# MMAThijssen/catfish

Hardware: AMD Instinct MI355X
Metric: signal samples/s classified (higher is better)
Workload: dtype f32

## Files before the change

### catfish_amd/csrc/catfish_hip.hip

```cpp
#include <hip/hip_runtime.h>
#include <stdint.h>
#include <string.h>
#include <stdio.h>
#include <vector>
#include <string>
#include <cmath>
#include <mutex>
#include <set>
#include <functional>

#include "../../include/catfish_hip.h"

typedef float f32x4 __attribute__((ext_vector_type(4)));
typedef float f32x2 __attribute__((ext_vector_type(2)));

#define CF_T 35
#define CF_H 64
#define CF_C 32
#define CF_TILE 16

#define MFMA16(a, b, c) __builtin_amdgcn_mfma_f32_16x16x4f32((a), (b), (c), 0, 0, 0)

#ifndef CF_ABLATE
#define CF_ABLATE 0
// ... 565 lines not shown
                cf_handoff_wait_agent(gflag - 1, lane, err);
            }
        }
        gru_tile<CIN, LAST, false, true>(lds, lane, dir, tile, X, Y, P, n_tiles, nullptr, nullptr, cf_dropout(), s_begin, s_end, ho, skip0);
        if (s_end < CF_T) {
            if (wave < nwaves - 1) cf_handoff_publish(flags + wave);
            else cf_handoff_publish_agent(gflag);
        }
    }
}

struct cf_fused_args {
    const float* w[3];
    const f32x4* x0;
    f32x4* y[2];
    float* p;
    unsigned* flags;
    int lds_floats;
    unsigned* err;
    int n_tiles;
    int groups;
    int n_layers;
    int cin0;
};

__device__ __forceinline__ bool cf_wait_flag(unsigned* flag) {
    for (int it = 0; it < 1000000; ++it) {
        if (__hip_atomic_load(flag, __ATOMIC_RELAXED, __HIP_MEMORY_SCOPE_AGENT) != 0u) return true;
        __builtin_amdgcn_s_sleep(16);
    }
    return false;
}

template <int CIN, bool LAST>
__device__ __forceinline__ void gru_fused_worker(float* lds, const cf_fused_args& a, int layer, int dir) {
    const f32x4* X = layer == 0 ? a.x0 : a.y[(layer - 1) & 1];
    f32x4* Y = a.y[layer & 1];
    gru_stage_weights<CIN>(lds, a.w[layer], dir);
    volatile int* slot = reinterpret_cast<volatile int*>(lds + a.lds_floats);
    unsigned* queue = a.flags + (size_t)a.n_layers * a.groups * 2 + layer * 2 + dir;
    const int lane = threadIdx.x & 63;
    const int wave = __builtin_amdgcn_readfirstlane(threadIdx.x >> 6);
    int group = 0;
    for (int iter = 0; iter <= a.groups && group < a.groups; ++iter) {
        if (threadIdx.x == 0) {
            const int g = (int)__hip_atomic_fetch_add(queue, 1u, __ATOMIC_RELAXED, __HIP_MEMORY_SCOPE_AGENT);
            if (layer > 0 && g < a.groups) {
                unsigned* f = a.flags + ((size_t)(layer - 1) * a.groups + g) * 2;
                if (!cf_wait_flag(f) || !cf_wait_flag(f + 1)) __hip_atomic_store(a.err, 1u, __ATOMIC_RELAXED, __HIP_MEMORY_SCOPE_SYSTEM);
                __builtin_amdgcn_fence(__ATOMIC_ACQUIRE, "agent");
                asm volatile("s_waitcnt vmcnt(0)" ::: "memory");
            }
            *slot = g;
        }
        __syncthreads();
        group = *slot;
        if (group < a.groups) {
            const int tile = group * 8 + wave;
            if (tile < a.n_tiles) gru_tile<CIN, LAST>(lds, lane, dir, tile, X, Y, a.p, a.n_tiles);
            asm volatile("s_waitcnt vmcnt(0)" ::: "memory");
            __syncthreads();
            if (!LAST && threadIdx.x == 0) {
                __builtin_amdgcn_fence(__ATOMIC_RELEASE, "agent");
                asm volatile("s_waitcnt vmcnt(0)" ::: "memory");
                __hip_atomic_store(a.flags + ((size_t)layer * a.groups + group) * 2 + dir, 1u, __ATOMIC_RELAXED,
                                   __HIP_MEMORY_SCOPE_AGENT);
            }
        }
    }
}

__global__ __launch_bounds__(512, 2) void gru_fused_kernel(cf_fused_args a) {
    extern __shared__ __attribute__((aligned(16))) float lds[];
    const int per_layer = gridDim.x / a.n_layers;
    const int layer = blockIdx.x / per_layer;
    const int dir = (blockIdx.x - layer * per_layer) & 1;
    const bool last = layer == a.n_layers - 1;
    if (layer == 0) {
        if (a.cin0 == 16) { if (last) gru_fused_worker<16, true>(lds, a, layer, dir); else gru_fused_worker<16, false>(lds, a, layer, dir); }
        else { if (last) gru_fused_worker<32, true>(lds, a, layer, dir); else gru_fused_worker<32, false>(lds, a, layer, dir); }
    } else {
        if (last) gru_fused_worker<128, true>(lds, a, layer, dir); else gru_fused_worker<128, false>(lds, a, layer, dir);
    }
}

#include "gru_coop.hpp"
#include "gru_train.hpp"
static_assert(gtb_pack_floats(32) == ((32 + CF_H) / 16 / 2) * 128 * 48 && gtb_pack_floats(128) == ((128 + CF_H) / 16 / 2) * 128 * 48,
              "gru_train_bwd_coop_kernel's PACK must equal gtb_pack_floats");
#include "gru_wgrad.hpp"
#include "res_train.hpp"
#include "train_step.hpp"

__global__ __launch_bounds__(256) void embed_kernel(const float* __restrict__ x_nat, f32x4* __restrict__ y_frag,
                                                    int64_t n_windows, int n_tiles) {
    const int64_t idx = (int64_t)blockIdx.x * 256 + threadIdx.x;
    if (idx >= (int64_t)n_tiles * CF_T * 64) return;
    const int lane = (int)(idx & 63);
    const int64_t tt = idx >> 6;
    const int t = (int)(tt % CF_T);
    const int64_t w = (tt / CF_T) * CF_TILE + (lane & 15);
    f32x4 v = {0.f, 0.f, 0.f, 0.f};
    if ((lane >> 4) == 0 && w < n_windows) v.x = x_nat[w * CF_T + t];
    y_frag[idx] = v;
}

#include "gru_bf16.hpp"
#include "gru_bf16_pipe.hpp"
#include "gru_bf16x3_pipe.hpp"

__global__ __launch_bounds__(256) void head_kernel(const float* __restrict__ P, const float* __restrict__ dense_bias, float* __restrict__ probs,
                                                   float* __restrict__ logits, int64_t n_windows, int n_tiles, int tile_shift, int raw) {
    const int64_t idx = (int64_t)blockIdx.x * 256 + threadIdx.x;
    if (idx >= n_windows * CF_T) return;
    const float bias = dense_bias[0];
// ... 225 lines not shown
        if (e_ != hipSuccess)                                                                      \
            return fail(CF_ERR_HIP, std::string(#expr) + ": " + hipGetErrorString(e_));           \
    } while (0)

enum { SLOT_RES_FIRST = 0, SLOT_RES, SLOT_GRU0, SLOT_GRU, SLOT_GRU_LAST, SLOT_HEAD, SLOT_POST, SLOT_NORM, SLOT_GRU_FUSED, SLOT_RES_STACK2 };
static const char* k_slot_names[CF_PROF_SLOTS] = {"res_block_first", "res_block",      "gru_layer_first", "gru_layer_mid",
                                                  "gru_layer_last",  "head",           "postprocess",     "normalize",       "gru_fused",
                                                  "res_stack2",      "unused",         "unused"};

struct cf_param_map;
static void pm_destroy(cf_param_map* pm);

struct cf_model {
    cf_hparams hp;
    int device = 0;
    int n_cu = 256;
    std::vector<float*> d_res;
    std::vector<float*> d_gru;
    std::vector<int> gru_cin;
    std::vector<char*> d_res_b;
    std::vector<char*> d_gru_b;
    int np = 0;
    float* d_dense_bias = nullptr;
    cf_param_map* pmap = nullptr;
    int64_t cap_windows = 0;
    int64_t cap_tiles = 0;
    struct Slot {
        float* d_a[2] = {nullptr, nullptr};
        float* d_y[2] = {nullptr, nullptr};
        float* d_p = nullptr;
        unsigned* d_flags = nullptr;
        float* d_hand = nullptr;
        unsigned* d_hand_flags = nullptr;
        hipStream_t stream = nullptr;
        hipEvent_t done = nullptr;
        int64_t last_windows = 0;
        bool last_res_fused = false;
    };
    std::vector<Slot> slots;
    cf_generic* gen = nullptr;
    int fuse = 0;
    float* d_xp = nullptr;
    int xp_tiles = 0;
    float* d_host_x = nullptr;
    float* d_host_p = nullptr;
    size_t host_stage_bytes = 0;
    unsigned* h_err = nullptr;
    unsigned* d_err = nullptr;
    hipEvent_t fork = nullptr;
    int64_t ws_bytes = 0;
    bool prof = false;
    int prof_every = 0;
    int64_t prof_calls = 0;
    struct Ev { hipEvent_t a, b; int slot; };
    std::vector<Ev> ev_pending;
    std::vector<hipEvent_t> ev_pool;
    double prof_ms[CF_PROF_SLOTS] = {0};
    int64_t prof_n[CF_PROF_SLOTS] = {0};
};

enum { CF_TERM_ZERO = 0, CF_TERM_RAW = 1, CF_TERM_KERN = 2, CF_TERM_BIAS = 3 };
enum { CF_K_ONE = 0, CF_K_GATE = 1, CF_K_CAND = 2 };
__host__ __device__ inline double cf_term_const(int c) { return c == CF_K_GATE ? CF_GATE_SCALE : (c == CF_K_CAND ? CF_CAND_SCALE : 1.0); }

__host__ __device__ inline double cf_bn_scale(float gamma, float var, float eps) {
#pragma clang fp contract(off)
// ... 210 lines not shown

static void pack_gru_dir(const cf_gru_dir& g, int cin, int cin_real, const float* dense_w ,
                         float* out) {
    cf_host_params P;
    P.t = {g.gates_kernel, g.gates_bias, g.candidate_kernel, g.candidate_bias, dense_w};
    HostSink e{P, out};
    pack_gru_dir(e, 0, gru_terms(0, CF_H), cin, cin_real, dense_w ? 4 : -1, 0);
}

static int upload(const std::vector<float>& host, float** dev) {
    HIP_TRY(hipMalloc((void**)dev, host.size() * sizeof(float)));
    HIP_TRY(hipMemcpy(*dev, host.data(), host.size() * sizeof(float), hipMemcpyHostToDevice));
    return CF_OK;
}

static bool gen_wanted(const cf_hparams* hp);
static int gen_build(cf_model* m, const cf_weights* w);
static void gen_destroy(cf_generic* g);
static hipError_t cf_optin_all();

extern "C" void cf_model_destroy(cf_model* m) {
    if (!m) return;
    (void)hipSetDevice(m->device);
    for (float* p : m->d_res) if (p) (void)hipFree(p);
    for (float* p : m->d_gru) if (p) (void)hipFree(p);
    for (char* p : m->d_gru_b) if (p) (void)hipFree(p);
    for (char* p : m->d_res_b) if (p) (void)hipFree(p);
    for (auto& sl : m->slots) {
        for (int i = 0; i < 2; ++i) { if (sl.d_a[i]) (void)hipFree(sl.d_a[i]); if (sl.d_y[i]) (void)hipFree(sl.d_y[i]); }
        if (sl.d_p) (void)hipFree(sl.d_p);
        if (sl.d_flags) (void)hipFree(sl.d_flags);
        if (sl.d_hand) (void)hipFree(sl.d_hand);
        if (sl.d_hand_flags) (void)hipFree(sl.d_hand_flags);
        if (sl.stream) (void)hipStreamDestroy(sl.stream);
        if (sl.done) (void)hipEventDestroy(sl.done);
    }
    gen_destroy(m->gen);
    pm_destroy(m->pmap);
    if (m->d_dense_bias) (void)hipFree(m->d_dense_bias);
    if (m->d_xp) (void)hipFree(m->d_xp);
    if (m->d_host_x) (void)hipFree(m->d_host_x);
    if (m->h_err) (void)hipHostFree(m->h_err);
    if (m->fork) (void)hipEventDestroy(m->fork);
    for (auto& e : m->ev_pending) { (void)hipEventDestroy(e.a); (void)hipEventDestroy(e.b); }
    for (auto& e : m->ev_pool) (void)hipEventDestroy(e);
    delete m;
}

extern "C" int cf_model_create(const cf_weights* w, const cf_hparams* hp, int device, cf_model** out) {
    if (!w || !hp || !out) return fail(CF_ERR_INVALID, "cf_model_create: null argument");
    *out = nullptr;
    if (hp->window != CF_T) return fail(CF_ERR_INVALID, "window must be 35 (rnn_class.py:27)");
    if (hp->n_layers < 1 || hp->n_layers_res < 0) return fail(CF_ERR_INVALID, "n_layers must be >= 1 and n_layers_res >= 0");
    const bool generic = gen_wanted(hp);
    if (!generic && hp->n_layers_res == 0 && hp->precision != CF_PREC_FP32)
        return fail(CF_ERR_INVALID, "the plain RNN type (n_layers_res = 0) is only built for CF_PREC_FP32");
    if ((hp->n_layers_res > 0 && !w->conv) || !w->gru || !w->dense_kernel || !w->dense_bias)
        return fail(CF_ERR_INVALID, "cf_weights has null members");
    int n_dev = 0;
    HIP_TRY(hipGetDeviceCount(&n_dev));
    if (device < 0 || device >= n_dev) return fail(CF_ERR_INVALID, "device index out of range");
    HIP_TRY(hipSetDevice(device));

    if (hp->precision < CF_PREC_FP32 || hp->precision > CF_PREC_BF16)
        return fail(CF_ERR_INVALID, "precision must be CF_PREC_FP32, CF_PREC_BF16X3 or CF_PREC_BF16");
    cf_model* m = new cf_model();
// ... 40 lines not shown
        if (w->gru[2 * l].cin != cin_real || w->gru[2 * l + 1].cin != cin_real) { rc = fail(CF_ERR_INVALID, "GRU layer input width mismatch"); break; }
        const bool last = l == hp->n_layers - 1;
        std::vector<float> blob((size_t)2 * gru_pack_floats(cin));
        HostSink e{P, blob.data()};
        for (int d = 0; d < 2; ++d)
            pack_gru_dir(e, (size_t)d * gru_pack_floats(cin), gru_terms(cf_tid_gru(hp->n_layers_res, l, d, 0), CF_H), cin, cin_real,
                         last ? cf_tid_dense(hp->n_layers_res, hp->n_layers, 0) : -1, d * CF_H);
        float* dptr = nullptr;
        rc = upload(blob, &dptr);
        m->d_gru.push_back(dptr);
        m->gru_cin.push_back(cin);
        if (rc == CF_OK && m->np > 0) {
            const size_t bytes = (size_t)gb_pack_bytes(cin, m->np);
            std::vector<char> bblob(2 * bytes, 0);
            for (int d = 0; d < 2; ++d)
                pack_gru_dir_bf16(w->gru[2 * l + d], cin, m->np, last ? w->dense_kernel + d * CF_H : nullptr, bblob.data() + d * bytes);
            char* bptr = nullptr;
            hipError_t e = hipMalloc((void**)&bptr, bblob.size());
            if (e == hipSuccess) e = hipMemcpy(bptr, bblob.data(), bblob.size(), hipMemcpyHostToDevice);
            if (e != hipSuccess) rc = fail(CF_ERR_HIP, std::string("bf16 weight upload: ") + hipGetErrorString(e));
            m->d_gru_b.push_back(bptr);
        }
    }
    if (rc == CF_OK) {
        int64_t cap = hp->max_windows_per_pass > 0 ? hp->max_windows_per_pass : 32768;
        cap = (cap + 2 * CF_TILE - 1) / (2 * CF_TILE) * (2 * CF_TILE);
        m->cap_windows = cap;
        m->cap_tiles = cap / CF_TILE;
        const size_t a_bytes = (size_t)m->cap_tiles * CF_T * 2 * 64 * sizeof(f32x4);
        const size_t y_bytes = (size_t)m->cap_tiles * CF_T * 8 * 64 * sizeof(f32x4);
        const cf_knobs knobs = cf_read_knobs();
        const size_t p_bytes = cf_dense_partial_floats(m->cap_tiles, m->n_cu) * sizeof(float);
        const size_t hand_bytes = cf_hand_bytes(m->n_cu);
        hipError_t e = hipSuccess;
        int n_slots = hp->n_streams > 0 ? hp->n_streams : 1;
        if (n_slots > 8) n_slots = 8;
        m->slots.resize(n_slots);
        for (auto& sl : m->slots) {
            for (int i = 0; i < 2 && e == hipSuccess; ++i) e = hipMalloc((void**)&sl.d_a[i], a_bytes);
            for (int i = 0; i < 2 && e == hipSuccess; ++i) e = hipMalloc((void**)&sl.d_y[i], y_bytes);
            if (e == hipSuccess) e = hipMalloc((void**)&sl.d_p, p_bytes);
            if (e == hipSuccess) e = hipMalloc((void**)&sl.d_flags, (size_t)3 * ((m->cap_tiles + 7) / 8) * 2 * sizeof(unsigned) + 64);
            if (e == hipSuccess && m->np == 0) e = hipMalloc((void**)&sl.d_hand, hand_bytes);
            if (e == hipSuccess && m->np == 0) e = hipMalloc((void**)&sl.d_hand_flags, cf_hand_flag_bytes(m->n_cu));
            if (e == hipSuccess && m->np == 0) e = hipMemset(sl.d_hand_flags, 0, cf_hand_flag_bytes(m->n_cu));
            if (e == hipSuccess && n_slots > 1) e = hipStreamCreateWithFlags(&sl.stream, hipStreamNonBlocking);
            if (e == hipSuccess && n_slots > 1) e = hipEventCreateWithFlags(&sl.done, hipEventDisableTiming);
        }
        if (e == hipSuccess && n_slots > 1) e = hipEventCreateWithFlags(&m->fork, hipEventDisableTiming);
        if (e == hipSuccess && n_slots == 1 && m->np == 0) {
            const int xpt = cf_hoist_limit(m->n_cu, m->cap_tiles, knobs);
            e = hipMalloc((void**)&m->d_xp, cf_xp_floats(xpt) * sizeof(float));
            if (e == hipSuccess) m->xp_tiles = xpt;
        }
        if (e == hipSuccess) e = hipHostMalloc((void**)&m->h_err, sizeof(unsigned), hipHostMallocMapped);
        if (e == hipSuccess) { *m->h_err = 0u; e = hipHostGetDevicePointer((void**)&m->d_err, m->h_err, 0); }
        m->fuse = cf_fuse_mode(m->np == 0 && hp->n_layers <= 3, hp->fuse_layers, knobs);
        if (e != hipSuccess) rc = fail(CF_ERR_NOMEM, std::string("workspace allocation: ") + hipGetErrorString(e));
        m->ws_bytes = (int64_t)n_slots * (int64_t)(2 * a_bytes + 2 * y_bytes + p_bytes + (m->np == 0 ? hand_bytes : 0));
    }
    if (rc == CF_OK) {
        hipError_t e = cf_optin_all();
        if (e != hipSuccess) rc = fail(CF_ERR_HIP, std::string("hipFuncSetAttribute(max dynamic LDS): ") + hipGetErrorString(e));
    }
    if (rc != CF_OK) { std::string keep = g_err; cf_model_destroy(m); g_err = keep; return rc; }
    *out = m;
    return CF_OK;
}

static int prof_begin(cf_model* m, int slot, hipStream_t s, size_t* idx) {
    if (!m->prof) return CF_OK;
    cf_model::Ev ev;
    ev.slot = slot;
    for (hipEvent_t* p : {&ev.a, &ev.b}) {
        if (!m->ev_pool.empty()) { *p = m->ev_pool.back(); m->ev_pool.pop_back(); }
        else HIP_TRY(hipEventCreate(p));
    }
    HIP_TRY(hipEventRecord(ev.a, s));
    m->ev_pending.push_back(ev);
    *idx = m->ev_pending.size() - 1;
    return CF_OK;
}
static int prof_end(cf_model* m, hipStream_t s, size_t idx) {
    if (!m->prof) return CF_OK;
    HIP_TRY(hipEventRecord(m->ev_pending[idx].b, s));
    return CF_OK;
}

template <int... Vs, class F>
static int cf_with(int v, F&& f) {
    int rc = CF_OK;
    const bool hit = ((v == Vs && ((rc = f(std::integral_constant<int, Vs>{})), true)) || ...);
    return hit ? rc : fail(CF_ERR_INVALID, "no kernel is built for template argument " + std::to_string(v));
}

struct cf_optin {
    hipError_t e = hipSuccess;
    void operator()(const void* f, int bytes) { if (e == hipSuccess) e = hipFuncSetAttribute(f, hipFuncAttributeMaxDynamicSharedMemorySize, bytes); }
};

template <int CIN> constexpr int k_gru_pack_bytes = gru_pack_floats(CIN) * 4;
template <int CIN> constexpr int k_gru_x_bytes = gru_x_floats(CIN) * 4;
static void optin_gru_layer(cf_optin& o) {
    for (int cin : {16, 32, 128})
        for (int last : {0, 1})
            cf_with<16, 32, 128>(cin, [&](auto C) { return cf_with<0, 1>(last, [&](auto L) {
                constexpr int CIN = decltype(C)::value;
                constexpr bool LAST = decltype(L)::value != 0;
                o((const void*)gru_layer_kernel<CIN, LAST>, cf_gru_layer_lds(k_gru_pack_bytes<CIN>));
                o((const void*)gru_layer_coop_kernel<CIN, LAST>, cf_gru_coop_lds(k_gru_pack_bytes<CIN>));
                return CF_OK;
            }); });
    o((const void*)gru_fused_kernel, cf_fused_lds(k_gru_pack_bytes<128>));
    o((const void*)gru_xproj_lds_kernel<32>, k_gru_x_bytes<32>);
    o((const void*)gru_xproj_lds_kernel<128>, k_gru_x_bytes<128>);
}

template <int CIN>
static void launch_xproj(cf_model* m, const cf_xproj_launch& xp, const float* wpack, const float* X, int n_tiles, hipStream_t s) {
    if (xp.lds_kernel)
        hipLaunchKernelGGL((gru_xproj_lds_kernel<CIN>), dim3(xp.grid_x, 2), dim3(256), xp.lds_bytes, s, wpack,
                           reinterpret_cast<const f32x4*>(X), reinterpret_cast<f32x4*>(m->d_xp), n_tiles, xp.chunks);
    else
        hipLaunchKernelGGL((gru_xproj_kernel<CIN>), dim3(xp.grid_x, 2), dim3(256), 0, s, wpack,
                           reinterpret_cast<const f32x4*>(X), reinterpret_cast<f32x4*>(m->d_xp), n_tiles, xp.chunks);
}

static int launch_gru(cf_model* m, const cf_knobs& k, int cin, bool last, const float* wpack, const float* X, float* Y, float* P, int n_tiles,
                      hipStream_t s, int slot, cf_gru_plan* ran = nullptr,
                      float* hand = nullptr,
                      unsigned* hand_flags = nullptr) {
    return cf_with<16, 32, 128>(cin, [&](auto C) { return cf_with<0, 1>(last, [&](auto L) {
        constexpr int CIN = decltype(C)::value;
        constexpr bool LAST = decltype(L)::value != 0;
        const cf_gru_plan p = cf_gru_plan_for(n_tiles, m->n_cu, CIN, k_gru_pack_bytes<CIN>, k_gru_x_bytes<CIN>, m->xp_tiles, hand && hand_flags, k);
        if (ran) *ran = p;
        size_t pi = 0;
        int rc = prof_begin(m, slot, s, &pi);
        if (rc != CF_OK) return rc;
        if (p.coop) {
            if (p.hoist) launch_xproj<CIN>(m, p.xproj, wpack, X, n_tiles, s);
            hipLaunchKernelGGL((gru_layer_coop_kernel<CIN, LAST>), dim3(p.gx, 2), dim3(p.waves * 64), p.lds_bytes, s, wpack,
                               reinterpret_cast<const f32x4*>(X), reinterpret_cast<f32x4*>(Y), P, n_tiles,
                               p.hoist ? reinterpret_cast<const f32x4*>(m->d_xp) : nullptr);
        } else {
            hipLaunchKernelGGL((gru_layer_kernel<CIN, LAST>), dim3(p.gx, 2), dim3(p.waves * 64), p.lds_bytes, s, wpack,
// ... 106 lines not shown
            if ((rc = prof_begin(m, b == 0 ? SLOT_RES_FIRST : SLOT_RES, s, &pi)) != CF_OK) return rc;
            bf16x8* dst = reinterpret_cast<bf16x8*>(sl.d_a[b & 1]);
            if (b == 0)
                hipLaunchKernelGGL((res_block_bf16_kernel<true, NP>), dim3(p.grid), dim3(256), p.lds_first, s, m->d_res_b[0], x, (const bf16x8*)nullptr,
                                   dst, n_windows, n_tiles32);
            else
                hipLaunchKernelGGL((res_block_bf16_kernel<false, NP>), dim3(p.grid), dim3(256), p.lds_other, s, m->d_res_b[b], (const float*)nullptr,
                                   reinterpret_cast<const bf16x8*>(sl.d_a[(b - 1) & 1]), dst, n_windows, n_tiles32);
            HIP_TRY(hipGetLastError());
            if ((rc = prof_end(m, s, pi)) != CF_OK) return rc;
        }
        return CF_OK;
    });
}

static int run_pass(cf_model* m, cf_model::Slot& sl, const float* x, int64_t n_windows, float* probs, float* logits, hipStream_t s) {
    const int n_tiles = (int)((n_windows + CF_TILE - 1) / CF_TILE);
    const int n_tiles32 = (int)((n_windows + 2 * CF_TILE - 1) / (2 * CF_TILE));
    const cf_knobs k = cf_read_knobs();
    int rc;
    size_t pi = 0;
    if ((rc = m->np > 0 ? run_res_bf16(m, sl, k, x, n_windows, n_tiles32, s) : run_res_fp32(m, sl, k, x, n_windows, n_tiles, s)) != CF_OK) return rc;
    if (m->hp.n_layers_res == 0) {
        if ((rc = prof_begin(m, SLOT_RES_FIRST, s, &pi)) != CF_OK) return rc;
        const int64_t n_el = (int64_t)n_tiles * CF_T * 64;
        hipLaunchKernelGGL(embed_kernel, dim3((unsigned)((n_el + 255) / 256)), dim3(256), 0, s, x,
                           reinterpret_cast<f32x4*>(sl.d_a[0]), n_windows, n_tiles);
        HIP_TRY(hipGetLastError());
        if ((rc = prof_end(m, s, pi)) != CF_OK) return rc;
    }
    const float* cur = m->hp.n_layers_res == 0 ? sl.d_a[0] : sl.d_a[(m->hp.n_layers_res - 1) & 1];
    cf_gru_plan last_gru = {};
    const int cin0 = m->hp.n_layers_res == 0 ? 16 : CF_C;
    if (cf_fuse_now(m->fuse, n_tiles, m->n_cu)) {
        cf_fused_args a;
        a.lds_floats = m->hp.n_layers > 1 ? gru_pack_floats(128) : gru_pack_floats(cin0);
        const cf_fused_plan p = cf_fused_plan_for(n_tiles, m->n_cu, m->hp.n_layers, a.lds_floats * 4);
        for (int l = 0; l < 3; ++l) a.w[l] = l < m->hp.n_layers ? m->d_gru[l] : nullptr;
        a.x0 = reinterpret_cast<const f32x4*>(cur);
        a.y[0] = reinterpret_cast<f32x4*>(sl.d_y[0]);
        a.y[1] = reinterpret_cast<f32x4*>(sl.d_y[1]);
        a.p = sl.d_p;
        a.flags = sl.d_flags;
        a.err = m->d_err;
        a.n_tiles = n_tiles;
        a.groups = p.groups;
        a.n_layers = m->hp.n_layers;
        a.cin0 = cin0;
        HIP_TRY(hipMemsetAsync(sl.d_flags, 0, ((size_t)a.n_layers * a.groups * 2 + (size_t)a.n_layers * 2) * sizeof(unsigned), s));
        if ((rc = prof_begin(m, SLOT_GRU_FUSED, s, &pi)) != CF_OK) return rc;
        hipLaunchKernelGGL(gru_fused_kernel, dim3((unsigned)p.grid), dim3(p.threads), p.lds_bytes, s, a);
        HIP_TRY(hipGetLastError());
        if ((rc = prof_end(m, s, pi)) != CF_OK) return rc;
    } else {
        for (int l = 0; l < m->hp.n_layers; ++l) {
            const bool last = l == m->hp.n_layers - 1;
            const int slot = last ? SLOT_GRU_LAST : (l == 0 ? SLOT_GRU0 : SLOT_GRU);
            float* y = sl.d_y[l & 1];
            rc = m->np > 0 ? launch_gru_bf16(m, k, m->gru_cin[l], last, m->d_gru_b[l], cur, y, sl.d_p, n_tiles32, s, slot)
                           : launch_gru(m, k, m->gru_cin[l], last, m->d_gru[l], cur, y, sl.d_p, n_tiles, s, slot, &last_gru, sl.d_hand, sl.d_hand_flags);
            if (rc != CF_OK) return rc;
            cur = y;
        }
    }
    if ((rc = prof_begin(m, SLOT_HEAD, s, &pi)) != CF_OK) return rc;
    const int64_t total = n_windows * CF_T;
    hipLaunchKernelGGL(head_kernel, dim3((unsigned)((total + 255) / 256)), dim3(256), 0, s, sl.d_p, m->d_dense_bias, probs, logits, n_windows,
                       m->np > 0 ? n_tiles32 : n_tiles, m->np > 0 ? 5 : 4, last_gru.raw_partials);
    HIP_TRY(hipGetLastError());
    if ((rc = prof_end(m, s, pi)) != CF_OK) return rc;
    sl.last_windows = n_windows;
    return CF_OK;
}

static const char* k_fused_timeout_msg = "a fused biGRU launch timed out waiting for a producer workgroup; its results are invalid "
                                         "(create the model with fuse_layers = -1)";

extern "C" int cf_check_error(cf_model* m) {
    if (!m) return fail(CF_ERR_INVALID, "cf_check_error: null model");
    if (m->h_err && *m->h_err) return fail(CF_ERR_HIP, k_fused_timeout_msg);
    return CF_OK;
}

extern "C" int cf_clear_error(cf_model* m) {
    if (!m) return fail(CF_ERR_INVALID, "cf_clear_error: null model");
    if (m->h_err) *m->h_err = 0u;
    HIP_TRY(hipSetDevice(m->device));
    HIP_TRY(hipDeviceSynchronize());
    for (auto& sl : m->slots)
        if (sl.d_hand_flags) HIP_TRY(hipMemset(sl.d_hand_flags, 0, cf_hand_flag_bytes(m->n_cu)));
    return CF_OK;
}

extern "C" int cf_launch_regimes(const cf_model* m, int64_t out[4]) {
    if (!m || !out) return fail(CF_ERR_INVALID, "cf_launch_regimes: null argument");
    out[0] = m->n_cu;
    if (m->gen) { out[1] = out[2] = out[3] = 0; return CF_OK; }
    out[1] = (int64_t)m->xp_tiles * CF_TILE;
    out[2] = m->np == 0 ? (int64_t)cf_coop_max_tiles(m->n_cu) * CF_TILE : 0;
    out[3] = m->fuse == 1 ? 1 : (m->fuse == 2 ? cf_fuse_auto_min_windows(m->n_cu) : 0);
    return CF_OK;
}

extern "C" int cf_infer_logits(cf_model* m, const float* x, int64_t n_windows, float* probs, float* logits, void* stream) {
    if (!m) return fail(CF_ERR_INVALID, "cf_infer: null model");
    if (n_windows < 0) return fail(CF_ERR_INVALID, "cf_infer: negative n_windows");
    if (n_windows == 0) return CF_OK;
    if (!x || (!probs && !logits)) return fail(CF_ERR_INVALID, "cf_infer: null buffer");
    if (m->h_err && *m->h_err) return fail(CF_ERR_HIP, k_fused_timeout_msg);
    HIP_TRY(hipSetDevice(m->device));
    hipStream_t s = reinterpret_cast<hipStream_t>(stream);
    m->prof = m->prof_every > 0 && (m->prof_calls++ % m->prof_every) == 0;
    if (m->gen) {
        for (int64_t off = 0; off < n_windows; off += m->cap_windows) {
            const int64_t n = std::min(m->cap_windows, n_windows - off);
            const int rc = gen_run_pass(m, x + off * CF_T, n, probs ? probs + off * CF_T : nullptr, logits ? logits + off * CF_T : nullptr, s);
            if (rc != CF_OK) return rc;
        }
        return CF_OK;
    }
    const int n_slots = (int)m->slots.size();
    int64_t chunk = m->cap_windows;
    if (n_slots > 1) {
// ... 827 lines not shown
```

### catfish_amd/csrc/gru_balance.hpp

```cpp
#pragma once

#if defined(__HIPCC__) || defined(__CUDACC__)
#define CF_BAL_HD __host__ __device__
#else
#define CF_BAL_HD
#endif

struct cf_gru_share {
    int head_tile, head_end;
    int whole_first, whole_count;
    int tail_tile, tail_begin;
    int interior;
    int steps;
};

CF_BAL_HD inline cf_gru_share cf_gru_balanced_share(int tiles, int nwaves, int wave, int T) {
    const int total = tiles * T;
    const int a = (int)((long long)wave * total / nwaves), b = (int)((long long)(wave + 1) * total / nwaves);
    cf_gru_share s;
    s.steps = b - a;
    s.tail_tile = a / T;
    s.tail_begin = a % T == 0 ? T : a % T;
    s.head_tile = b / T;
    s.head_end = b % T;
// ... 52 lines not shown
    int worst = 0;
    long long rem = 0;
    for (int b = 0; b < gx; ++b) {
        int big = 0;
        for (int w = 0; w < nwaves; ++w) {
            rem += r;
            if (rem >= W) { rem -= W; ++big; }
        }
        const int v = per_simd * q + (big < per_simd ? big : per_simd);
        if (v > worst) worst = v;
    }
    return worst * wg_per_cu;
}

struct cf_gru_choice {
    int balance;
    int gx;
    int load;
};
CF_BAL_HD inline cf_gru_choice cf_gru_choose(int n_tiles, int gx, int gx_one, int nwaves, int wg_per_cu, int T, int forced) {
    const bool two = gx_one > 0 && gx > gx_one;
    const int load_rr = cf_gru_grid_load(n_tiles, gx, nwaves, wg_per_cu, T, 0);
    const int load_bal = cf_gru_grid_load(n_tiles, gx, nwaves, wg_per_cu, T, 1);
    const int load_one = two ? cf_gru_grid_load(n_tiles, gx_one, nwaves, 1, T, 1) : -1;
    const int load_grid = cf_gru_gridwide_load(n_tiles, gx, nwaves, wg_per_cu, T);
    const int load_grid_one = two ? cf_gru_gridwide_load(n_tiles, gx_one, nwaves, 1, T) : -1;
    cf_gru_choice c = {0, gx, load_rr};
    if (forced < 0 ? (load_bal >= 0 && load_bal < c.load) : (forced >= 1 && load_bal >= 0)) { c.balance = 1; c.load = load_bal; }
    if (forced < 0 ? (load_one >= 0 && load_one < c.load) : (forced >= 2 && load_one >= 0)) { c.balance = 1; c.gx = gx_one; c.load = load_one; }
    if (forced < 0 ? (load_grid >= 0 && load_grid < c.load) : (forced == 3 && load_grid >= 0)) { c.balance = 2; c.gx = gx; c.load = load_grid; }
    if (forced < 0 ? (load_grid_one >= 0 && load_grid_one < c.load) : (forced == 3 && load_grid_one >= 0)) { c.balance = 2; c.gx = gx_one; c.load = load_grid_one; }
    return c;
}
```

### catfish_amd/csrc/tuned_launch.hpp

```cpp
#pragma once

#include <algorithm>
#include <climits>
#include <cstddef>
#include <cstdint>

#ifndef CF_T
#define CF_T 35
#define CF_TILE 16
#endif
#define CF_GRU_MAX_WAVES 8
#define CF_COOP_XCH_FLOATS (2 * 4 * 64 * 4 + 4 * 64)
#define CF_COOP_BWD_XCH_FLOATS (3 * 4 * 64 * 4)
#include "gru_balance.hpp"

constexpr int CF_LDS_LIMIT = 160 * 1024;
enum { CF_GRU_SCHED_MASK = 3, CF_GRU_RUN_ZERO_PRODUCTS = 4 };

constexpr int CF_KNOB_UNSET = INT_MIN;
struct cf_knobs {
    int coop = CF_KNOB_UNSET, waves = CF_KNOB_UNSET, gru_balance = CF_KNOB_UNSET, gru_gx = CF_KNOB_UNSET, gru_zero_products = CF_KNOB_UNSET;
    int xproj_lds = CF_KNOB_UNSET, xproj_chunks = CF_KNOB_UNSET, hoist_tiles = CF_KNOB_UNSET, fuse = CF_KNOB_UNSET;
    int bf16_waves = CF_KNOB_UNSET, bf16_wgs = CF_KNOB_UNSET, bf16_pipe = CF_KNOB_UNSET;
    int res_fuse = CF_KNOB_UNSET, res_tpw = CF_KNOB_UNSET, res_chunks = CF_KNOB_UNSET, dx_chunks = CF_KNOB_UNSET;
// ... 91 lines not shown
    int lds_bytes;
    int raw_partials;
};
inline cf_gru_plan cf_gru_plan_for(int n_tiles, int n_cu, int cin, int pack_bytes, int x_bytes, int hoist_tiles, bool has_hand, const cf_knobs& k) {
    cf_gru_plan p = {};
    p.load = -1;
    if (cf_use_coop(n_tiles, n_cu, k)) {
        p.coop = p.raw_partials = 1;
        p.waves = 4;
        p.gx = cf_coop_gx(n_tiles, n_cu);
        p.hoist = cin >= 32 && n_tiles <= hoist_tiles;
        if (p.hoist) p.xproj = cf_xproj_launch_for(n_tiles, n_cu, cin, x_bytes, k);
        p.lds_bytes = cf_gru_coop_lds(pack_bytes);
        return p;
    }
    const int gx_env = cf_forced_gx(n_cu, k);
    p.waves = gx_env > 0 ? 8 : k.waves > 0 ? std::min(k.waves, 8) : (k.ablate_four_waves ? 4 : cf_pick_waves(2 * n_tiles, n_cu));
    const int groups = cf_ceil_div(n_tiles, p.waves);
    p.per_dir = cf_half_cus(n_cu);
    if (pack_bytes <= CF_LDS_LIMIT / 2) p.per_dir *= 2;
    p.gx = std::min(groups, p.per_dir);
    if (gx_env > 0) p.gx = std::min(gx_env, groups);
    p.balance = CF_GRU_RUN_ZERO_PRODUCTS;
    if (has_hand) {
        p.wg_per_cu = std::max(1, cf_ceil_div(2 * p.gx, n_cu));
        p.gx_one = gx_env > 0 ? 0 : cf_half_cus(n_cu);
        const cf_gru_choice c = cf_gru_choose(n_tiles, p.gx, p.gx_one, p.waves, p.wg_per_cu, CF_T, cf_knob_or(k.gru_balance, -1));
        p.balance = c.balance | (cf_knob_or(k.gru_zero_products, 0) != 0 ? CF_GRU_RUN_ZERO_PRODUCTS : 0);
        p.gx = c.gx;
        p.load = c.load;
    }
    p.lds_bytes = cf_gru_layer_lds(pack_bytes);
    return p;
}

struct cf_gru_bf16_plan {
    int pipe;
    int waves, gx, lds_bytes;
};
inline cf_gru_bf16_plan cf_gru_bf16_plan_for(int n_tiles32, int n_cu, int np, int pack_bytes, const cf_knobs& k) {
    cf_gru_bf16_plan p;
    p.pipe = cf_knob_or(k.bf16_pipe, 1) != 0;
    p.lds_bytes = pack_bytes;
    p.waves = k.bf16_waves > 0 ? std::min(k.bf16_waves, 8) : cf_pick_waves(2 * n_tiles32, n_cu);
    int per_dir = cf_half_cus(n_cu);
    if (np == 2 && p.pipe) {
        p.waves = std::min(p.waves, 4);
    } else if (pack_bytes <= CF_LDS_LIMIT / 2) {
        per_dir *= 2;
    }
    if (k.bf16_wgs > 0) per_dir = k.bf16_wgs;
    p.gx = std::min(cf_ceil_div(n_tiles32, p.waves), per_dir);
    return p;
}

constexpr int CF_XS_BYTES = CF_TILE * CF_T * 4;
struct cf_res_plan {
    int split;
    int chunks, waves, grid;
    int lds_first, lds_other;
    int fused;
    int stack_chunks, stack_waves, stack_grid, stack_lds;
};
constexpr int cf_res_stack2_lds(int pack_first_bytes, int pack_other_bytes, int waves) { return pack_first_bytes + pack_other_bytes + waves * CF_XS_BYTES; }
inline cf_res_plan cf_res_plan_for(int n_tiles, int n_cu, int n_blocks, int pack_first_bytes, int pack_other_bytes, const cf_knobs& k) {
    cf_res_plan p = {};
// ... 88 lines not shown
```

Before: 348.4 million.

## Add chained multi-layer GRU kernel with per-producer epoch flags and fused head

Adds a single persistent kernel that runs all GRU layers and both directions at once. Each workgroup handles a fixed balanced share and waits only on the specific producer workgroups of the layer below, using epoch-tagged done flags, instead of a layer-wide barrier or separate launches. The last layer also computes the sigmoid head inline once both directions for a tile have arrived, which removes the separate head kernel launch. It is enabled automatically for fp32 models with up to three layers when the gridwide balanced plan applies. The cost is extra sync workspace and spin-waits, and it depends on every layer's workgroups being co-resident on the device.

```diff
diff --git a/catfish_amd/csrc/catfish_hip.hip b/catfish_amd/csrc/catfish_hip.hip
--- a/catfish_amd/csrc/catfish_hip.hip
+++ b/catfish_amd/csrc/catfish_hip.hip
@@ -621,6 +621,14 @@
     return false;
 }
 
+__device__ __forceinline__ bool cf_wait_flag_is(unsigned* flag, unsigned value) {
+    for (int it = 0; it < 1000000; ++it) {
+        if (__hip_atomic_load(flag, __ATOMIC_RELAXED, __HIP_MEMORY_SCOPE_AGENT) == value) return true;
+        __builtin_amdgcn_s_sleep(16);
+    }
+    return false;
+}
+
 template <int CIN, bool LAST>
 __device__ __forceinline__ void gru_fused_worker(float* lds, const cf_fused_args& a, int layer, int dir) {
     const f32x4* X = layer == 0 ? a.x0 : a.y[(layer - 1) & 1];
@@ -670,6 +678,134 @@
         else { if (last) gru_fused_worker<32, true>(lds, a, layer, dir); else gru_fused_worker<32, false>(lds, a, layer, dir); }
     } else {
         if (last) gru_fused_worker<128, true>(lds, a, layer, dir); else gru_fused_worker<128, false>(lds, a, layer, dir);
+    }
+}
+
+struct cf_chain_args {
+    const float* w[3];
+    const f32x4* x0;
+    f32x4* y[2];
+    float* p;
+    f32x4* hand;
+    unsigned* gflags;
+    unsigned* done;
+    unsigned* arrive;
+    unsigned* epoch;
+    const float* dense_bias;
+    float* probs;
+    unsigned* err;
+    long long n_windows;
+    int n_tiles, gx, n_layers, cin0;
+    int skip0;
+    int ablate;
+};
+
+template <int CIN, bool LAST>
+__device__ __forceinline__ void gru_chain_worker(float* lds, const cf_chain_args& a, int layer, int dir, int b) {
+    const f32x4* X = layer == 0 ? a.x0 : a.y[(layer - 1) & 1];
+    f32x4* Y = a.y[layer & 1];
+    gru_stage_weights<CIN>(lds, a.w[layer], dir);
+    unsigned* flags = reinterpret_cast<unsigned*>(lds + gru_pack_floats(CIN));
+    if (threadIdx.x <= CF_GRU_MAX_WAVES) flags[threadIdx.x] = 0u;
+    auto set_now = [&]() { return __hip_atomic_load(a.epoch, __ATOMIC_RELAXED, __HIP_MEMORY_SCOPE_AGENT) + 1u; };
+    const int lane = threadIdx.x & 63;
+    const int wave = __builtin_amdgcn_readfirstlane(threadIdx.x >> 6);
+    const int nwaves = blockDim.x >> 6;
+    if (layer > 0 && threadIdx.x == 0 && !(a.ablate & 4)) {
+        const cf_gru_wg_range r = cf_gru_chain_producers(a.n_tiles, a.gx, nwaves, CF_T, b, 0, 0);
+        unsigned* below = a.done + (size_t)(layer - 1) * 2 * a.gx;
+        const unsigned want = set_now();
+        bool ok = true;
+        for (int i = 0; i < r.count; ++i) {
+            const int pb = (r.first + i) % a.gx;
+            ok = cf_wait_flag_is(below + pb, want) && ok;
+            ok = cf_wait_flag_is(below + a.gx + pb, want) && ok;
+        }
+        if (!ok) __hip_atomic_store(a.err, 1u, __ATOMIC_RELAXED, __HIP_MEMORY_SCOPE_SYSTEM);
+        __builtin_amdgcn_fence(__ATOMIC_ACQUIRE, "agent");
+        asm volatile("s_waitcnt vmcnt(0)" ::: "memory");
+    }
+    __syncthreads();
+    const cf_gru_share sh = cf_gru_balanced_share(a.n_tiles, a.gx * nwaves, b * nwaves + wave, CF_T);
+    const int has_head = sh.head_end > 0;
+    const int n_pieces = has_head + sh.whole_count + (sh.tail_begin < CF_T);
+    const size_t row = (size_t)(layer * 2 + dir) * a.gx + b;
+    f32x4* slots = a.hand + row * CF_GRU_MAX_WAVES * 4 * 64;
+    unsigned* gflag = a.gflags + row;
+    const float bias = LAST ? a.dense_bias[0] : 0.f;
+    for (int i = 0; i < n_pieces; ++i) {
+        int tile, s_begin = 0, s_end = CF_T;
+        f32x4* ho = nullptr;
+        if (i < has_head) {
+            tile = sh.head_tile; s_end = sh.head_end; ho = slots + wave * 4 * 64;
+        } else if (i < has_head + sh.whole_count) {
+            tile = sh.whole_first + (i - has_head);
+        } else {
+            tile = sh.tail_tile; s_begin = sh.tail_begin;
+            if (wave > 0) {
+                ho = slots + (wave - 1) * 4 * 64;
+                cf_handoff_wait(flags + (wave - 1), lane, a.err);
+            } else {
+                ho = slots - (CF_GRU_MAX_WAVES - (nwaves - 1)) * 4 * 64;
+                cf_handoff_wait_agent(gflag - 1, lane, a.err);
+            }
+        }
+        gru_tile<CIN, LAST, false, true>(lds, lane, dir, tile, X, Y, a.p, a.n_tiles, nullptr, nullptr, cf_dropout(), s_begin, s_end, ho,
+                                         a.skip0 != 0);
+        if (s_end < CF_T) {
+            if (wave < nwaves - 1) cf_handoff_publish(flags + wave);
+            else cf_handoff_publish_agent(gflag);
+        } else if (LAST && a.probs) {
+            asm volatile("s_waitcnt vmcnt(0)" ::: "memory");
+            __builtin_amdgcn_fence(__ATOMIC_RELEASE, "agent");
+            asm volatile("s_waitcnt vmcnt(0)" ::: "memory");
+            unsigned before = 0u;
+            if (lane == 0) before = __hip_atomic_fetch_add(a.arrive + tile, 1u, __ATOMIC_RELAXED, __HIP_MEMORY_SCOPE_AGENT);
+            if (__builtin_amdgcn_readfirstlane(before) & 1u) {
+                __builtin_amdgcn_fence(__ATOMIC_ACQUIRE, "agent");
+                asm volatile("s_waitcnt vmcnt(0)" ::: "memory");
+                const float* pf = a.p + (int64_t)tile * CF_T * 16;
+                const float* pb = a.p + ((int64_t)a.n_tiles + tile) * CF_T * 16;
+                for (int j = lane; j < CF_TILE * CF_T; j += 64) {
+                    const int wl = j / CF_T, t = j - wl * CF_T;
+                    if ((int64_t)tile * CF_TILE + wl < a.n_windows) {
+                        const float z = pf[t * 16 + wl] + pb[t * 16 + wl] + bias;
+                        a.probs[(int64_t)tile * CF_TILE * CF_T + j] = 1.0f / (1.0f + expf(-z));
+                    }
+                }
+            }
+        }
+    }
+    if (!LAST && !(a.ablate & 2)) {
+        asm volatile("s_waitcnt vmcnt(0)" ::: "memory");
+        __builtin_amdgcn_fence(__ATOMIC_RELEASE, "agent");
+        asm volatile("s_waitcnt vmcnt(0)" ::: "memory");
+    }
+    if (lane == 0) {
+        const unsigned through = __hip_atomic_fetch_add(flags + CF_GRU_MAX_WAVES, 1u, __ATOMIC_ACQ_REL, __HIP_MEMORY_SCOPE_WORKGROUP);
+        if (through == (unsigned)nwaves - 1u) {
+            const unsigned set = set_now();
+            if constexpr (!LAST) __hip_atomic_store(a.done + row, set, __ATOMIC_RELAXED, __HIP_MEMORY_SCOPE_AGENT);
+            const unsigned out = __hip_atomic_fetch_add(a.epoch + 1, 1u, __ATOMIC_RELAXED, __HIP_MEMORY_SCOPE_AGENT);
+            if (out == gridDim.x - 1u) {
+                __hip_atomic_store(a.epoch + 1, 0u, __ATOMIC_RELAXED, __HIP_MEMORY_SCOPE_AGENT);
+                __hip_atomic_store(a.epoch, set, __ATOMIC_RELAXED, __HIP_MEMORY_SCOPE_AGENT);
+            }
+        }
+    }
+}
+
+__global__ __launch_bounds__(512, 2) void gru_chain_kernel(cf_chain_args a) {
+    extern __shared__ __attribute__((aligned(16))) float lds[];
+    const int layer = blockIdx.x / (2 * a.gx);
+    const int rest = blockIdx.x - layer * 2 * a.gx;
+    const int dir = rest / a.gx, b = rest - dir * a.gx;
+    const bool last = layer == a.n_layers - 1;
+    if (layer == 0) {
+        if (a.cin0 == 16) { if (last) gru_chain_worker<16, true>(lds, a, layer, dir, b); else gru_chain_worker<16, false>(lds, a, layer, dir, b); }
+        else { if (last) gru_chain_worker<32, true>(lds, a, layer, dir, b); else gru_chain_worker<32, false>(lds, a, layer, dir, b); }
+    } else {
+        if (last) gru_chain_worker<128, true>(lds, a, layer, dir, b); else gru_chain_worker<128, false>(lds, a, layer, dir, b);
     }
 }
 
@@ -961,6 +1097,8 @@
         unsigned* d_flags = nullptr;
         float* d_hand = nullptr;
         unsigned* d_hand_flags = nullptr;
+        float* d_chain_hand = nullptr;
+        unsigned* d_chain_sync = nullptr;
         hipStream_t stream = nullptr;
         hipEvent_t done = nullptr;
         int64_t last_windows = 0;
@@ -1237,6 +1375,8 @@
         if (sl.d_flags) (void)hipFree(sl.d_flags);
         if (sl.d_hand) (void)hipFree(sl.d_hand);
         if (sl.d_hand_flags) (void)hipFree(sl.d_hand_flags);
+        if (sl.d_chain_hand) (void)hipFree(sl.d_chain_hand);
+        if (sl.d_chain_sync) (void)hipFree(sl.d_chain_sync);
         if (sl.stream) (void)hipStreamDestroy(sl.stream);
         if (sl.done) (void)hipEventDestroy(sl.done);
     }
@@ -1343,6 +1483,7 @@
         const cf_knobs knobs = cf_read_knobs();
         const size_t p_bytes = cf_dense_partial_floats(m->cap_tiles, m->n_cu) * sizeof(float);
         const size_t hand_bytes = cf_hand_bytes(m->n_cu);
+        const bool chain_ws = m->np == 0 && hp->n_layers <= 3;
         hipError_t e = hipSuccess;
         int n_slots = hp->n_streams > 0 ? hp->n_streams : 1;
         if (n_slots > 8) n_slots = 8;
@@ -1355,6 +1496,9 @@
             if (e == hipSuccess && m->np == 0) e = hipMalloc((void**)&sl.d_hand, hand_bytes);
             if (e == hipSuccess && m->np == 0) e = hipMalloc((void**)&sl.d_hand_flags, cf_hand_flag_bytes(m->n_cu));
             if (e == hipSuccess && m->np == 0) e = hipMemset(sl.d_hand_flags, 0, cf_hand_flag_bytes(m->n_cu));
+            if (e == hipSuccess && chain_ws) e = hipMalloc((void**)&sl.d_chain_hand, cf_chain_hand_bytes(m->n_cu));
+            if (e == hipSuccess && chain_ws) e = hipMalloc((void**)&sl.d_chain_sync, cf_chain_sync_bytes(m->n_cu, m->cap_tiles));
+            if (e == hipSuccess && chain_ws) e = hipMemset(sl.d_chain_sync, 0, cf_chain_sync_bytes(m->n_cu, m->cap_tiles));
             if (e == hipSuccess && n_slots > 1) e = hipStreamCreateWithFlags(&sl.stream, hipStreamNonBlocking);
             if (e == hipSuccess && n_slots > 1) e = hipEventCreateWithFlags(&sl.done, hipEventDisableTiming);
         }
@@ -1368,7 +1512,8 @@
         if (e == hipSuccess) { *m->h_err = 0u; e = hipHostGetDevicePointer((void**)&m->d_err, m->h_err, 0); }
         m->fuse = cf_fuse_mode(m->np == 0 && hp->n_layers <= 3, hp->fuse_layers, knobs);
         if (e != hipSuccess) rc = fail(CF_ERR_NOMEM, std::string("workspace allocation: ") + hipGetErrorString(e));
-        m->ws_bytes = (int64_t)n_slots * (int64_t)(2 * a_bytes + 2 * y_bytes + p_bytes + (m->np == 0 ? hand_bytes : 0));
+        m->ws_bytes = (int64_t)n_slots * (int64_t)(2 * a_bytes + 2 * y_bytes + p_bytes + (m->np == 0 ? hand_bytes : 0) +
+                                                 (chain_ws ? cf_chain_hand_bytes(m->n_cu) : 0));
     }
     if (rc == CF_OK) {
         hipError_t e = cf_optin_all();
@@ -1423,6 +1568,7 @@
                 return CF_OK;
             }); });
     o((const void*)gru_fused_kernel, cf_fused_lds(k_gru_pack_bytes<128>));
+    o((const void*)gru_chain_kernel, cf_chain_lds(k_gru_pack_bytes<128>));
     o((const void*)gru_xproj_lds_kernel<32>, k_gru_x_bytes<32>);
     o((const void*)gru_xproj_lds_kernel<128>, k_gru_x_bytes<128>);
 }
@@ -1595,7 +1741,45 @@
     const float* cur = m->hp.n_layers_res == 0 ? sl.d_a[0] : sl.d_a[(m->hp.n_layers_res - 1) & 1];
     cf_gru_plan last_gru = {};
     const int cin0 = m->hp.n_layers_res == 0 ? 16 : CF_C;
-    if (cf_fuse_now(m->fuse, n_tiles, m->n_cu)) {
+    const char* chain_env = cf_knob("CATFISH_CHAIN");
+    const bool fuse_now = cf_fuse_now(m->fuse, n_tiles, m->n_cu);
+    const cf_chain_plan ch = cf_chain_plan_for(n_tiles, m->n_cu, m->hp.n_layers, cin0, cin0 == 16 ? k_gru_pack_bytes<16> : k_gru_pack_bytes<32>,
+                                               k_gru_pack_bytes<128>, cin0 == 16 ? k_gru_x_bytes<16> : k_gru_x_bytes<32>, k_gru_x_bytes<128>,
+                                               m->xp_tiles, m->np == 0 && sl.d_chain_hand && sl.d_chain_sync, logits != nullptr, m->prof,
+                                               chain_env ? atoi(chain_env) : CF_KNOB_UNSET, CF_CHAIN_AUTO && !fuse_now, k);
+    if (ch.on) {
+        cf_chain_args a;
+        for (int l = 0; l < 3; ++l) a.w[l] = l < m->hp.n_layers ? m->d_gru[l] : nullptr;
+        a.x0 = reinterpret_cast<const f32x4*>(cur);
+        a.y[0] = reinterpret_cast<f32x4*>(sl.d_y[0]);
+        a.y[1] = reinterpret_cast<f32x4*>(sl.d_y[1]);
+        a.p = sl.d_p;
+        a.hand = reinterpret_cast<f32x4*>(sl.d_chain_hand);
+        a.epoch = sl.d_chain_sync;
+        a.gflags = sl.d_chain_sync + 4;
+        a.done = a.gflags + cf_chain_max_rows(m->n_cu);
+        a.arrive = a.done + cf_chain_max_rows(m->n_cu);
+        a.dense_bias = m->d_dense_bias;
+        a.probs = probs;
+        a.err = m->d_err;
+        a.n_windows = n_windows;
+        a.n_tiles = n_tiles;
+        a.gx = ch.gx;
+        a.n_layers = m->hp.n_layers;
+        a.cin0 = cin0;
+        a.skip0 = ch.skip0;
+        const char* abl_env = cf_knob("CATFISH_CHAIN_ABLATE");
+        a.ablate = abl_env ? atoi(abl_env) : 0;
+        if (a.ablate & 1) a.probs = nullptr;
+        hipLaunchKernelGGL(gru_chain_kernel, dim3((unsigned)ch.grid), dim3(ch.threads), ch.lds_bytes, s, a);
+        HIP_TRY(hipGetLastError());
+        sl.last_windows = n_windows;
+        if (!(a.ablate & 1)) return CF_OK;
+        hipLaunchKernelGGL(head_kernel, dim3((unsigned)((n_windows * CF_T + 255) / 256)), dim3(256), 0, s, sl.d_p, m->d_dense_bias, probs, logits, n_windows,
+                           n_tiles, 4, 0);
+        return CF_OK;
+    }
+    if (fuse_now) {
         cf_fused_args a;
         a.lds_floats = m->hp.n_layers > 1 ? gru_pack_floats(128) : gru_pack_floats(cin0);
         const cf_fused_plan p = cf_fused_plan_for(n_tiles, m->n_cu, m->hp.n_layers, a.lds_floats * 4);
@@ -1652,6 +1836,8 @@
     HIP_TRY(hipDeviceSynchronize());
     for (auto& sl : m->slots)
         if (sl.d_hand_flags) HIP_TRY(hipMemset(sl.d_hand_flags, 0, cf_hand_flag_bytes(m->n_cu)));
+    for (auto& sl : m->slots)
+        if (sl.d_chain_sync) HIP_TRY(hipMemset(sl.d_chain_sync, 0, cf_chain_sync_bytes(m->n_cu, m->cap_tiles)));
     return CF_OK;
 }
 
diff --git a/catfish_amd/csrc/gru_balance.hpp b/catfish_amd/csrc/gru_balance.hpp
--- a/catfish_amd/csrc/gru_balance.hpp
+++ b/catfish_amd/csrc/gru_balance.hpp
@@ -108,3 +108,22 @@
     if (forced < 0 ? (load_grid_one >= 0 && load_grid_one < c.load) : (forced == 3 && load_grid_one >= 0)) { c.balance = 2; c.gx = gx_one; c.load = load_grid_one; }
     return c;
 }
+
+struct cf_gru_wg_range { int first, count; };
+CF_BAL_HD inline cf_gru_wg_range cf_gru_chain_producers(int n_tiles, int gx, int nwaves, int T, int b, int rot_cons, int rot_prod) {
+    const long long W = (long long)gx * nwaves, total = (long long)n_tiles * T;
+    const long long rc = ((rot_cons % W) + W) % W, rp = ((rot_prod % W) + W) % W;
+    const long long s0 = ((long long)b * nwaves + rc) % W;
+    const long long s1 = (s0 + nwaves - 1) % W;
+    const long long x_lo = (s0 * total / W) / T * T;
+    const long long x_hi = (((s1 + 1) * total / W - 1) / T) * T + T - 1;
+    const long long p_lo = ((x_lo + 1) * W - 1) / total, p_hi = ((x_hi + 1) * W - 1) / total;
+    long long n_shares = s1 < s0 ? (W - p_lo) + p_hi + 1 : p_hi - p_lo + 1;
+    if (n_shares > W) n_shares = W;
+    const long long g0 = (p_lo - rp + W) % W;
+    cf_gru_wg_range r;
+    r.first = (int)(g0 / nwaves);
+    const long long n = (g0 + n_shares - 1) / nwaves - r.first + 1;
+    r.count = (int)(n > gx ? gx : n);
+    return r;
+}
diff --git a/catfish_amd/csrc/tuned_launch.hpp b/catfish_amd/csrc/tuned_launch.hpp
--- a/catfish_amd/csrc/tuned_launch.hpp
+++ b/catfish_amd/csrc/tuned_launch.hpp
@@ -147,6 +147,34 @@
     }
     p.lds_bytes = cf_gru_layer_lds(pack_bytes);
     return p;
+}
+
+constexpr bool CF_CHAIN_AUTO = true;
+constexpr int cf_chain_lds(int pack_bytes) { return pack_bytes + (CF_GRU_MAX_WAVES + 1) * 4; }
+inline int cf_chain_max_rows(int n_cu) { return 3 * 2 * cf_half_cus(n_cu); }
+inline size_t cf_chain_hand_bytes(int n_cu) { return (size_t)cf_chain_max_rows(n_cu) * CF_GRU_MAX_WAVES * 4 * 64 * 16; }
+inline size_t cf_chain_sync_bytes(int n_cu, int64_t cap_tiles) { return ((size_t)4 + 2 * cf_chain_max_rows(n_cu) + (size_t)cap_tiles) * sizeof(unsigned); }
+struct cf_chain_plan { int on, gx, grid, threads, lds_bytes, skip0; };
+inline cf_chain_plan cf_chain_plan_for(int n_tiles, int n_cu, int n_layers, int cin0, int pack0_bytes, int pack_bytes, int x0_bytes, int x_bytes,
+                                       int hoist_tiles, bool fp32, bool want_logits, bool events, int chain, bool auto_on, const cf_knobs& k) {
+    cf_chain_plan c = {};
+    const bool wanted = cf_knob_set(chain) ? chain != 0 : auto_on;
+    if (!wanted || !fp32 || n_layers < 1 || n_layers > 3 || want_logits || events) return c;
+    int lds = 0;
+    for (int l = 0; l < n_layers; ++l) {
+        const cf_gru_plan p = cf_gru_plan_for(n_tiles, n_cu, l == 0 ? cin0 : 128, l == 0 ? pack0_bytes : pack_bytes, l == 0 ? x0_bytes : x_bytes,
+                                              hoist_tiles, true, k);
+        if (p.coop || (p.balance & CF_GRU_SCHED_MASK) != 2 || p.waves != CF_GRU_MAX_WAVES || (l > 0 && p.gx != c.gx)) return c;
+        c.gx = p.gx;
+        c.skip0 = !(p.balance & CF_GRU_RUN_ZERO_PRODUCTS);
+        lds = std::max(lds, cf_chain_lds(l == 0 ? pack0_bytes : pack_bytes));
+    }
+    if (!cf_gru_gridwide_ok(n_tiles, c.gx, CF_GRU_MAX_WAVES) || n_layers * 2 * c.gx > cf_chain_max_rows(n_cu)) return c;
+    c.on = 1;
+    c.grid = n_layers * 2 * c.gx;
+    c.threads = CF_GRU_MAX_WAVES * 64;
+    c.lds_bytes = lds;
+    return c;
 }
 
 struct cf_gru_bf16_plan {
```

Result: slower. 339.8 million (-2.5%).
